# emstoudenmire/TNML

Hardware: AMD Instinct MI355X
Metric: two-site bond updates/sec (higher is better)
Workload: dtype f64; 1 GPU; fixedL N=784, maxm=120, 60000 images (BASELINE config 3: its 60 000 images on 1 GPU instead of 8), Npass=4, lambda=0.001, minm=120, fp64 throughout; random-init W at m=maxm; timed bonds 405..202 (consecutive interior bonds, Label-carrying shiftE on each, m=119); global_images=60000, sites=784, maxm=120, parallelism=dp1 (image sharding + RCCL all-reduce), rccl_ranks=1

## Files before the change

### tnml_amd/csrc/kernels_res.hip

```cpp
#include "tnml_internal.h"

typedef double f64x4r __attribute__((ext_vector_type(4)));

#define FR_TI 32
#define FR_ROWS(NKA) (4 * (NKA) + 4)
#define FR_EIS(NKA) (FR_ROWS(NKA) * FR_TI)
#define FR_LDS_DOUBLES_N(NKA) (2 * FR_EIS(NKA) + 2 * 64 * FR_TI + 2 * 4 * TNML_NL * FR_TI)
#define FR_LDS_DOUBLES FR_LDS_DOUBLES_N(30)

static __device__ __forceinline__ void fr_barrier() {
    asm volatile("s_waitcnt lgkmcnt(0)" ::: "memory");
    __builtin_amdgcn_s_barrier();
    asm volatile("" ::: "memory");
}

template <int PS, int PK, int ABL, int NKA = 30, bool GEN = false, int NST = 8>
__global__ __launch_bounds__(768) void k_fwd_res(FwdResArgs A) {
    static_assert(GEN || NKA == 30, "the constant-extent form is the 120 x 120 bond");
    static_assert(NST == 8 || (NST == 4 && GEN), "four or eight streaming steps per tile");
    constexpr int EIS = FR_EIS(NKA);
    const int mI = GEN ? A.mI : 120, mO = GEN ? A.mO : 120, Kp = GEN ? A.Kp : 240, Np = GEN ? A.Np : 240;
    extern __shared__ __attribute__((aligned(16))) double fr_lds[];
    double* EIs = fr_lds;
    double* Us = EIs + 2 * EIS;
    double* red = Us + 2 * 64 * FR_TI;
    const int tid = threadIdx.x, lane = tid & 63, wid = __builtin_amdgcn_readfirstlane(tid >> 6);
    const int b = blockIdx.x;
    const int half = (b >> 3) & 1, pair = (b & 7) + 8 * (b >> 4), npairs = gridDim.x >> 1;
    const int NTp = A.NTp;
    const int T = Np >> 4, T0 = (T + 1) >> 1;
    const int Th = half ? T - T0 : T0;
    const int qb = half ? 8 * T0 : 0;
    const int niter = (A.ntiles - pair + npairs - 1) / npairs;

    if (wid < 8) {
        const int w = wid;
        const bool act = w < Th;
        const int ct = (half ? T0 : 0) + w;
        double me[NKA], mo[NKA];
        {
            const int g = lane >> 4, i = lane & 15;
            const int col = 2 * (8 * ct + (i & 7)) + (i >> 3);
#pragma unroll
            for (int ks = 0; ks < NKA; ++ks) {
                const bool in = act && 2 * (4 * ks + g) + 1 < Kp;
                me[ks] = in ? A.M[(size_t)(2 * (4 * ks + g)) * Np + col] : 0.;
                mo[ks] = in ? A.M[(size_t)(2 * (4 * ks + g) + 1) * Np + col] : 0.;
            }
        }
        fr_barrier();
        long long t_mma = 0, t_epi = 0, t_bar = 0;
        const long long wc0 = ABL == 5 ? (long long)wall_clock64() : 0;
        for (int it = 0; it < niter + 2; ++it) {
            const long long c0 = ABL == 5 ? clock64() : 0;
            long long c1 = c0, c2 = c0;
            if (it < niter && act) {
                const double* Eb = EIs + (it & 1) * EIS;
                double* Ub = Us + (it & 1) * 64 * FR_TI;
                int ln = lane;
                asm volatile("" : "+v"(ln));
                int g = ln >> 4, i = ln & 15;
                const double* ep0 = Eb + g * FR_TI + 16 * (g & 1) + i;
                const double* ep1 = Eb + g * FR_TI + 16 * ((g & 1) ^ 1) + i;
                f64x4r ce0 = {0., 0., 0., 0.}, co0 = {0., 0., 0., 0.}, ce1 = {0., 0., 0., 0.}, co1 = {0., 0., 0., 0.};
                double a0 = ep0[0], b0 = ep1[0], a1 = ep0[4 * FR_TI], b1 = ep1[4 * FR_TI];
                __builtin_amdgcn_sched_group_barrier(0x100, 4, 0);
#pragma unroll
                for (int ks = 0; ks < (ABL == 2 ? 1 : NKA); ++ks) {
                    const double xa = a0, xb = b0;
                    a0 = a1; b0 = b1;
                    if (ks + 2 < NKA) { a1 = ep0[4 * (ks + 2) * FR_TI]; b1 = ep1[4 * (ks + 2) * FR_TI]; __builtin_amdgcn_sched_group_barrier(0x100, 2, 0); }
                    ce0 = __builtin_amdgcn_mfma_f64_16x16x4f64(me[ks], xa, ce0, 0, 0, 0);
                    co0 = __builtin_amdgcn_mfma_f64_16x16x4f64(mo[ks], xa, co0, 0, 0, 0);
                    ce1 = __builtin_amdgcn_mfma_f64_16x16x4f64(me[ks], xb, ce1, 0, 0, 0);
                    co1 = __builtin_amdgcn_mfma_f64_16x16x4f64(mo[ks], xb, co1, 0, 0, 0);
                    __builtin_amdgcn_sched_group_barrier(0x008, 4, 0);
                    if (PS > 0 && ks % PK == PK - 1) { __builtin_amdgcn_s_sleep(PS); __builtin_amdgcn_sched_barrier(0); }
                }
                if (ABL == 5) c1 = clock64();
                ln = lane;
                asm volatile("" : "+v"(ln));
                g = ln >> 4; i = ln & 15;
#pragma unroll
                for (int grp = 0; grp < 2; ++grp) {
                    const double pI0 = Eb[(4 * NKA) * FR_TI + 16 * grp + i], pI1 = Eb[(4 * NKA + 1) * FR_TI + 16 * (grp ^ 1) + i];
                    const double pO0 = Eb[(4 * NKA + 2) * FR_TI + 16 * grp + i], pO1 = Eb[(4 * NKA + 3) * FR_TI + 16 * (grp ^ 1) + i];
                    const f64x4r ce = grp ? ce1 : ce0, co = grp ? co1 : co0;
#pragma unroll
                    for (int e = 0; e < 2; ++e) {
                        const double t0 = fma(pI1, co[e], pI0 * ce[e]), t1 = fma(pI1, co[e + 2], pI0 * ce[e + 2]);
                        const double v = fma(pO1, t1, pO0 * t0);
                        Ub[(8 * w + g + 4 * e) * FR_TI + 16 * grp + i] = v;
                    }
                }
                if (ABL == 5) c2 = clock64();
            }
            fr_barrier();
            if (ABL == 5) { const long long c3 = clock64(); t_mma += c1 - c0; t_epi += c2 - c1; t_bar += c3 - c2; }
        }
        if (ABL == 5 && A.dbg && blockIdx.x < 16 && lane == 0) { long long* d = A.dbg + (blockIdx.x * 12 + wid) * 4; d[0] = t_mma; d[1] = t_epi; d[2] = t_bar; d[3] = (long long)wall_clock64() - wc0; }
    } else {
        __builtin_amdgcn_s_setprio(3);
        const int sw = wid - 8;
        const int img = lane & 31, qs = lane >> 5;
        const int nk = Th;
        const unsigned lds0 = (unsigned)(size_t)((__attribute__((address_space(3))) char*)fr_lds);
        const int xcol = 2 * ((lane & 15) ^ (((lane >> 4) & 1) << 3));
        const double* const phr = ((lane >> 4) < 2 ? A.phiI : A.phiO) + (size_t)((lane >> 4) & 1) * NTp + xcol;
        const double* const eir = A.EI + (size_t)(lane >> 4) * NTp + xcol;
        const int gb = GEN ? (mI - 1) >> 2 : NKA;
        const int rb = 4 * gb + (lane >> 4) < mI ? 4 * gb + (lane >> 4) : mI - 1;
        const double* const eib = A.EI + (size_t)rb * NTp + xcol;
        auto x_stage = [&](int tile, int buf) {
#pragma unroll
            for (int r = 0; r < 8; ++r) {
                int grp = sw + 4 * r;
                const double* src;
                if constexpr (GEN) {
                    if (grp > NKA) grp -= NKA + 1;
                    if (grp > NKA) grp -= NKA + 1;
                    src = (grp == NKA ? phr : (grp < gb ? eir + (size_t)(4 * grp) * NTp : (grp == gb ? eib : eir))) + (size_t)tile * FR_TI;
                } else {
                    grp = r < 7 ? sw + 4 * r : (sw < 2 ? sw + 28 : (sw == 2 ? 30 : 3));
                    src = (grp == 30 ? phr : eir + (size_t)(4 * grp) * NTp) + (size_t)tile * FR_TI;
                }
                const unsigned dst = lds0 + (unsigned)((buf * EIS + 4 * grp * FR_TI) * sizeof(double));
                unsigned keep;
                asm volatile("s_mov_b32 %0, m0\n\ts_mov_b32 m0, %2\n\ts_nop 0\n\tglobal_load_lds_dwordx4 %1, off\n\ts_mov_b32 m0, %0"
                             : "=&s"(keep) : "v"(src), "s"(dst) : "memory");
            }
        };
        const double* ELw = A.EL + (size_t)(qb + 2 * sw) * NTp;
        const unsigned eoff = (unsigned)(((size_t)qs * NTp + img) * sizeof(double));
        const unsigned uoff = (unsigned)((2 * sw + qs) * FR_TI + img);
        size_t roff[8]; bool same[8];
#pragma unroll
        for (int k = 0; k < 8; ++k) {
            const int q0 = qb + 8 * k + 2 * sw;
            const bool real = k < nk && q0 < mO;
            roff[k] = real ? (size_t)(8 * k) * NTp : (size_t)0 - (size_t)qb * NTp;
            same[k] = GEN && real && q0 + 1 >= mO;
        }
        const unsigned eoff0 = (unsigned)(img * sizeof(double));
        double ea[TNML_NL], eb[TNML_NL], ec[TNML_NL], ed[TNML_NL];
        auto s_load = [&](int tile, int k, double (&e)[TNML_NL]) {
            const unsigned vo = same[k] ? eoff0 : eoff;
#pragma unroll
            for (int l = 0; l < TNML_NL; ++l) {
                const double* bp = ELw + (size_t)tile * FR_TI + (size_t)l * A.EL_lstride + roff[k];
                if (ABL == 1) e[l] = 1.0;
                else asm volatile("global_load_dwordx2 %0, %1, %2 nt" : "=v"(e[l]) : "v"(vo), "s"(bp) : "memory");
            }
        };
#define FR_WAIT(N, e) asm volatile("s_waitcnt vmcnt(" #N ")" : "+v"(e[0]), "+v"(e[1]), "+v"(e[2]), "+v"(e[3]), "+v"(e[4]), "+v"(e[5]), "+v"(e[6]), "+v"(e[7]), "+v"(e[8]), "+v"(e[9]) :: "memory")
        auto label_dot = [&](int tile, int ntile, const double* Ub, double* rb, auto&& mid) {
            double px[TNML_NL];
#pragma unroll
            for (int l = 0; l < TNML_NL; ++l) px[l] = 0.;
            auto s_use = [&](int k, const double (&e)[TNML_NL], bool on) {
                double u = Ub[8 * k * FR_TI + uoff];
                if (!on) u = 0.;
#pragma unroll
                for (int l = 0; l < TNML_NL; ++l) px[l] = fma(e[l], u, px[l]);
            };
#define FR_FENCE() do { asm volatile("" : "+v"(px[0]), "+v"(px[1]), "+v"(px[2]), "+v"(px[3]), "+v"(px[4]), "+v"(px[5]), "+v"(px[6]), "+v"(px[7]), "+v"(px[8]), "+v"(px[9]) :: "memory"); \
                        __builtin_amdgcn_sched_barrier(0); } while (0)
            if constexpr (NST == 8) {
                FR_WAIT(30, ea); s_use(0, ea, nk > 0); FR_FENCE(); s_load(tile, 4, ea);
                FR_WAIT(30, eb); s_use(1, eb, nk > 1); FR_FENCE(); s_load(tile, 5, eb);
                FR_WAIT(30, ec); s_use(2, ec, nk > 2); FR_FENCE(); s_load(tile, 6, ec);
                FR_WAIT(30, ed); s_use(3, ed, nk > 3); FR_FENCE(); s_load(tile, 7, ed);
                mid();
                FR_WAIT(38, ea); s_use(4, ea, nk > 4); FR_FENCE(); s_load(ntile, 0, ea);
                FR_WAIT(38, eb); s_use(5, eb, nk > 5); FR_FENCE(); s_load(ntile, 1, eb);
                FR_WAIT(38, ec); s_use(6, ec, nk > 6); FR_FENCE(); s_load(ntile, 2, ec);
                FR_WAIT(38, ed); s_use(7, ed, nk > 7); FR_FENCE(); s_load(ntile, 3, ed);
            } else {
                FR_WAIT(30, ea); s_use(0, ea, nk > 0); FR_FENCE(); s_load(ntile, 0, ea);
                FR_WAIT(30, eb); s_use(1, eb, nk > 1); FR_FENCE(); s_load(ntile, 1, eb);
                mid();
                FR_WAIT(38, ec); s_use(2, ec, nk > 2); FR_FENCE(); s_load(ntile, 2, ec);
                FR_WAIT(38, ed); s_use(3, ed, nk > 3); FR_FENCE(); s_load(ntile, 3, ed);
            }
#undef FR_FENCE
#pragma unroll
            for (int l = 0; l < TNML_NL; ++l) {
                px[l] += __shfl_xor(px[l], 32);
                if (qs == 0) rb[(sw * TNML_NL + l) * FR_TI + img] = px[l];
            }
        };
        auto finalize = [&](int tile, const double* rb) {
            if (sw == 0) {
#pragma unroll
                for (int l2 = 0; l2 < TNML_NL / 2; ++l2) {
                    const int l = 2 * l2 + qs;
                    const double s = ((rb[(0 * TNML_NL + l) * FR_TI + img] + rb[(1 * TNML_NL + l) * FR_TI + img]) + rb[(2 * TNML_NL + l) * FR_TI + img]) + rb[(3 * TNML_NL + l) * FR_TI + img];
                    A.Ppart[((size_t)half * TNML_NL + l) * NTp + (size_t)tile * FR_TI + img] = s;
                }
            }
        };
        x_stage(pair, 0);
        asm volatile("s_waitcnt vmcnt(0)" ::: "memory");
        fr_barrier();
        x_stage(niter > 1 ? pair + npairs : pair, 1);
        s_load(pair, 0, ea); s_load(pair, 1, eb); s_load(pair, 2, ec); s_load(pair, 3, ed);
        asm volatile("s_waitcnt vmcnt(40)" ::: "memory");
        fr_barrier();
        long long t_dot = 0, t_bar = 0;
        for (int it = 1; it <= niter; ++it) {
            const long long c0 = ABL == 5 ? clock64() : 0;
            const int tile = pair + (it - 1) * npairs;
            label_dot(tile, it < niter ? tile + npairs : tile, Us + ((it - 1) & 1) * 64 * FR_TI, red + (it & 1) * 4 * TNML_NL * FR_TI, [&]() {
                x_stage(it + 1 < niter ? pair + (it + 1) * npairs : tile, (it + 1) & 1);
                if (it >= 2) finalize(pair + (it - 2) * npairs, red + ((it - 1) & 1) * 4 * TNML_NL * FR_TI);
            });
            if constexpr (NST == 8) asm volatile("s_waitcnt vmcnt(40)" ::: "memory");
            else                    asm volatile("s_waitcnt vmcnt(20)" ::: "memory");
            const long long c1 = ABL == 5 ? clock64() : 0;
            fr_barrier();
            if (ABL == 5) { const long long c2 = clock64(); t_dot += c1 - c0; t_bar += c2 - c1; }
        }
        if (ABL == 5 && A.dbg && blockIdx.x < 16 && lane == 0) { long long* d = A.dbg + (blockIdx.x * 12 + wid) * 4; d[0] = t_dot; d[1] = 0; d[2] = t_bar; d[3] = niter; }
        asm volatile("s_waitcnt vmcnt(0)" ::: "memory");
        finalize(pair + (niter - 1) * npairs, red + (niter & 1) * 4 * TNML_NL * FR_TI);
        fr_barrier();
#undef FR_WAIT
    }
}

#define SR_TI 64

template <int NKS, int NG, int NSK>
static __device__ __forceinline__ void sr_groups(const double* Eb, const double (&me)[NKS], const double (&mo)[NKS], int lane, unsigned sl, double (&ob)[16]) {
    int ln = lane;
    asm volatile("" : "+v"(ln));
    int g = ln >> 4;
    const double* ep[NG];
    f64x4r ce[NG], co[NG];
    double x0[NG];
#pragma unroll
    for (int j = 0; j < NG; ++j) {
        ep[j] = Eb + g * SR_TI + ((sl >> (8 * j)) & 63);
        ce[j] = f64x4r{0., 0., 0., 0.}; co[j] = f64x4r{0., 0., 0., 0.};
    }
#pragma unroll
    for (int j = 0; j < NG; ++j) x0[j] = ep[j][0];
    __builtin_amdgcn_sched_group_barrier(0x100, NG, 0);
#pragma unroll
    for (int ks = 0; ks < NKS; ++ks) {
        double xa[NG];
#pragma unroll
        for (int j = 0; j < NG; ++j) xa[j] = x0[j];
        if (ks + 1 < NKS) {
#pragma unroll
            for (int j = 0; j < NG; ++j) x0[j] = ep[j][4 * (ks + 1) * SR_TI];
            __builtin_amdgcn_sched_group_barrier(0x100, NG, 0);
        }
#pragma unroll
        for (int j = 0; j < NG; ++j) {
            ce[j] = __builtin_amdgcn_mfma_f64_16x16x4f64(me[ks], xa[j], ce[j], 0, 0, 0);
            if (j >= NSK) co[j] = __builtin_amdgcn_mfma_f64_16x16x4f64(mo[ks], xa[j], co[j], 0, 0, 0);
        }
        __builtin_amdgcn_sched_group_barrier(0x008, 2 * NG - NSK, 0);
    }
#pragma unroll
    for (int j = 0; j < NG; ++j) {
        const int im = (sl >> (8 * j)) & 63;
        const double pI0 = Eb[(4 * NKS) * SR_TI + im];
        if (j < NSK) {
#pragma unroll
            for (int e = 0; e < 4; ++e) ob[4 * j + e] = pI0 * ce[j][e];
        } else {
            const double pI1 = Eb[(4 * NKS + 1) * SR_TI + im];
#pragma unroll
            for (int e = 0; e < 4; ++e) ob[4 * j + e] = fma(pI1, co[j][e], pI0 * ce[j][e]);
        }
    }
    asm volatile("" ::: "memory");
    __builtin_amdgcn_sched_barrier(0);
}

template <int NKS, bool ZS>
__global__ __launch_bounds__(512) void k_shift_res(ShiftResArgs A) {
    constexpr int ROWS = 4 * NKS + 2;
    constexpr int NP = 2 * NKS + 1;
    extern __shared__ __attribute__((aligned(16))) double sr_lds[];
    const int tid = threadIdx.x, lane = tid & 63, w = __builtin_amdgcn_readfirstlane(tid >> 6);
    const int NTp = A.NTp, tpl = NTp / SR_TI;
    const int G = gridDim.x;
    const int niter = (A.ntiles - (int)blockIdx.x + G - 1) / G;
    const unsigned lds0 = __builtin_amdgcn_readfirstlane((unsigned)(size_t)((__attribute__((address_space(3))) char*)sr_lds));
    const unsigned doff = (unsigned)(((size_t)(lane >> 5) * NTp + 2 * (lane & 31)) * sizeof(double));
    auto dma16 = [&](const double* base, unsigned voff, unsigned dst) {
        unsigned keep;
        asm volatile("s_mov_b32 %0, m0\n\ts_mov_b32 m0, %2\n\ts_nop 0\n\tglobal_load_lds_dwordx4 %1, %3\n\ts_mov_b32 m0, %0" : "=&s"(keep) : "v"(voff), "s"(dst), "s"(base) : "memory");
    };
    const unsigned doff0 = (unsigned)((2 * (lane & 31)) * sizeof(double));
    auto stage = [&](int t, int buf) {
        const int l = t / tpl, n0 = (t - l * tpl) * SR_TI;
        const double* eb = A.EI + (size_t)l * A.EI_lstride + n0;
#pragma unroll
        for (int r = 0; r < 8; ++r) {
            int p = w + 8 * r;
            if (p >= NP) p -= NP;
            if (p >= NP) p -= NP;
            const int r0 = 2 * p < A.mI ? 2 * p : 0;
            dma16(p == NP - 1 ? A.phiI + n0 : eb + (size_t)r0 * NTp, (p != NP - 1 && 2 * p == A.mI - 1) ? doff0 : doff, lds0 + (unsigned)((buf * ROWS * SR_TI + 2 * p * SR_TI) * sizeof(double)));
        }
    };
    const int CT = A.Np >> 4;
    const bool split = CT <= 4;
    const int ct = split ? (w & 3) : w;
    const bool act = ct < CT;
    const bool do0 = !split || w < 4, do1 = !split || w >= 4;
    double me[NKS], mo[NKS];
    {
        const int g = lane >> 4, i = lane & 15;
#pragma unroll
        for (int ks = 0; ks < NKS; ++ks) {
            const bool in = act && 2 * (4 * ks + g) + 1 < A.Kp;
            me[ks] = in ? A.M[(size_t)(2 * (4 * ks + g)) * A.Np + 16 * ct + i] : 0.;
            mo[ks] = in ? A.M[(size_t)(2 * (4 * ks + g) + 1) * A.Np + 16 * ct + i] : 0.;
        }
    }
    if (niter > 0) stage(blockIdx.x, 0);
    asm volatile("s_waitcnt vmcnt(0)" ::: "memory");
    fr_barrier();
    if constexpr (ZS) {
        auto slots = [&](int t, int ln) {
            const uint8_t* o = A.ord + (size_t)(t % tpl) * SR_TI + (ln & 15);
            return (unsigned)o[0] | (unsigned)o[16] << 8 | (unsigned)o[32] << 16 | (unsigned)o[48] << 24;
        };
        auto put = [&](int t, int ln, unsigned psl, const double (&ob)[16]) {
            const int l = t / tpl, n0 = (t - l * tpl) * SR_TI, g = ln >> 4;
            double* op = A.out + (size_t)l * A.out_lstride + (size_t)(16 * ct + g) * NTp + n0;
#pragma unroll
            for (int q = 0; q < 16; ++q) {
                const int y = 16 * ct + g + 4 * (q & 3);
                if (y < A.mO && (q < 8 || !split)) op[(size_t)(4 * (q & 3)) * NTp + ((psl >> (8 * (q >> 2))) & 63)] = ob[q];
            }
        };
        unsigned sl = 0, sln = 0, psl = 0;
        if (niter > 0) sl = slots(blockIdx.x, lane);
        double ob[16];
        for (int it = 0; it < niter; ++it) {
            const int t = blockIdx.x + it * G;
            int ln = lane;
            asm volatile("" : "+v"(ln));
            if (act && it > 0) put(t - G, ln, psl, ob);
            if (it + 1 < niter) { stage(t + G, (it + 1) & 1); sln = slots(t + G, ln); }
            const double* Eb = sr_lds + (it & 1) * ROWS * SR_TI;
            if (act) {
                const int s = __builtin_amdgcn_readfirstlane((int)(((sl >> 6) & 3) | ((sl >> 12) & 4)));
                if (!split) {
                    switch (s) {
                        case 0:  sr_groups<NKS, 4, 0>(Eb, me, mo, lane, sl, ob); break;
                        case 1:  sr_groups<NKS, 4, 1>(Eb, me, mo, lane, sl, ob); break;
                        case 2:  sr_groups<NKS, 4, 2>(Eb, me, mo, lane, sl, ob); break;
                        case 3:  sr_groups<NKS, 4, 3>(Eb, me, mo, lane, sl, ob); break;
                        default: sr_groups<NKS, 4, 4>(Eb, me, mo, lane, sl, ob); break;
                    }
                    psl = sl;
                } else {
                    const int s2 = w < 4 ? (s < 2 ? s : 2) : (s > 2 ? s - 2 : 0);
                    psl = w < 4 ? sl : sl >> 16;
                    switch (s2) {
                        case 0:  sr_groups<NKS, 2, 0>(Eb, me, mo, lane, psl, ob); break;
                        case 1:  sr_groups<NKS, 2, 1>(Eb, me, mo, lane, psl, ob); break;
                        default: sr_groups<NKS, 2, 2>(Eb, me, mo, lane, psl, ob); break;
                    }
                }
            }
            asm volatile("s_waitcnt vmcnt(0)" : "+v"(sln) :: "memory");
            sl = sln;
            fr_barrier();
        }
        if (act && niter > 0) put(blockIdx.x + (niter - 1) * G, lane, psl, ob);
        return;
    }
    double ob[8];
    double* obp = nullptr;
    for (int it = 0; it < niter; ++it) {
        const int t = blockIdx.x + it * G;
        const int l = t / tpl, n0 = (t - l * tpl) * SR_TI;
        int ln = lane;
        asm volatile("" : "+v"(ln));
        int g = ln >> 4, i = ln & 15;
        if (obp) {
#pragma unroll
            for (int q = 0; q < 8; ++q) { const int y = 16 * ct + g + 4 * (q & 3); if (y < A.mO) obp[(size_t)(4 * (q & 3)) * NTp + 16 * (q >> 2)] = ob[q]; }
        }
        if (it + 1 < niter) stage(t + G, (it + 1) & 1);
        const double* Eb = sr_lds + (it & 1) * ROWS * SR_TI;
        double* op = A.out + (size_t)l * A.out_lstride + (size_t)(16 * ct + g) * NTp + n0 + i;
        if (act) {
#pragma unroll
            for (int pass = 0; pass < 2; ++pass) {
                if (pass == 0 ? !do0 : !do1) continue;
                const double* ep0 = Eb + g * SR_TI + 32 * pass + i;
                const double* ep1 = ep0 + 16;
                f64x4r ce0 = {0., 0., 0., 0.}, co0 = {0., 0., 0., 0.}, ce1 = {0., 0., 0., 0.}, co1 = {0., 0., 0., 0.};
                double a0 = ep0[0], b0 = ep1[0], a1 = ep0[4 * SR_TI], b1 = ep1[4 * SR_TI];
                __builtin_amdgcn_sched_group_barrier(0x100, 4, 0);
#pragma unroll
                for (int ks = 0; ks < NKS; ++ks) {
                    const double xa = a0, xb = b0;
                    a0 = a1; b0 = b1;
                    if (ks + 2 < NKS) { a1 = ep0[4 * (ks + 2) * SR_TI]; b1 = ep1[4 * (ks + 2) * SR_TI]; __builtin_amdgcn_sched_group_barrier(0x100, 2, 0); }
                    ce0 = __builtin_amdgcn_mfma_f64_16x16x4f64(me[ks], xa, ce0, 0, 0, 0);
                    co0 = __builtin_amdgcn_mfma_f64_16x16x4f64(mo[ks], xa, co0, 0, 0, 0);
                    ce1 = __builtin_amdgcn_mfma_f64_16x16x4f64(me[ks], xb, ce1, 0, 0, 0);
                    co1 = __builtin_amdgcn_mfma_f64_16x16x4f64(mo[ks], xb, co1, 0, 0, 0);
                    __builtin_amdgcn_sched_group_barrier(0x008, 4, 0);
                }
                ln = lane;
                asm volatile("" : "+v"(ln));
                g = ln >> 4; i = ln & 15;
#pragma unroll
                for (int grp = 0; grp < 2; ++grp) {
                    const double pI0 = Eb[(4 * NKS) * SR_TI + 32 * pass + 16 * grp + i], pI1 = Eb[(4 * NKS + 1) * SR_TI + 32 * pass + 16 * grp + i];
#pragma unroll
                    for (int e = 0; e < 4; ++e) {
                        const double v = fma(pI1, grp ? co1[e] : co0[e], pI0 * (grp ? ce1[e] : ce0[e]));
                        if (pass == 0) { if (16 * ct + g + 4 * e < A.mO) op[(size_t)(4 * e) * NTp + 16 * grp] = v; }
                        else ob[4 * grp + e] = v;
                    }
                }
                asm volatile("" ::: "memory");
                __builtin_amdgcn_sched_barrier(0);
            }
            if (do1) obp = op + 32;
        }
        asm volatile("s_waitcnt vmcnt(0)" ::: "memory");
        fr_barrier();
    }
    if (obp) {
        const int g = lane >> 4;
#pragma unroll
        for (int q = 0; q < 8; ++q) { const int y = 16 * ct + g + 4 * (q & 3); if (y < A.mO) obp[(size_t)(4 * (q & 3)) * NTp + 16 * (q >> 2)] = ob[q]; }
    }
}

static const int sr_nks_list[] = {12, 16, 18, 20, 22, 24, 26, 28, 30};
static int sr_nks_for(int mI) {
    for (int v : sr_nks_list) if (4 * v >= mI) return v;
    return 0;
}
bool shift_res_applies(int mI, int mO) { return mI >= 33 && sr_nks_for(mI) != 0 && mO >= 1 && mO <= 128; }

template <int NKS>
static int shift_res_go(tnml_ctx* c, const ShiftResArgs& a, int grid) {
    const size_t lds = sizeof(double) * 2 * (4 * NKS + 2) * SR_TI;
    if (!c->attr_sr[NKS]) {
        if (hipFuncSetAttribute(reinterpret_cast<const void*>(k_shift_res<NKS, false>), hipFuncAttributeMaxDynamicSharedMemorySize, (int)lds) != hipSuccess ||
            hipFuncSetAttribute(reinterpret_cast<const void*>(k_shift_res<NKS, true>), hipFuncAttributeMaxDynamicSharedMemorySize, (int)lds) != hipSuccess)
            return tnml_fail(c, "shift_res: cannot reserve %zu bytes of LDS", lds);
        c->attr_sr[NKS] = true;
    }
    ProfScope ps(c, KC_FGEMM_SHIFT);
    if (a.ord && a.nz) hipLaunchKernelGGL((k_shift_res<NKS, true>), dim3(grid), dim3(512), lds, c->stream, a);
    else               hipLaunchKernelGGL((k_shift_res<NKS, false>), dim3(grid), dim3(512), lds, c->stream, a);
    return 0;
}
int launch_shift_res(tnml_ctx* c, const ShiftResArgs& a_in) {
    ShiftResArgs a = a_in;
    if (a.NTp % SR_TI) return tnml_fail(c, "shift_res: image count not a multiple of %d", SR_TI);
    if (((size_t)a.L * a.EI_lstride) * sizeof(double) >= ((size_t)1 << 32)) return tnml_fail(c, "shift_res: environment larger than 4 GB (32-bit lane offsets)");
    if (!shift_res_applies(a.mI, a.mO) || a.Np % 16 || a.Np < a.mO || a.Np > 128) return tnml_fail(c, "shift_res: bond dimensions %d x %d (packed %d) not served", a.mI, a.mO, a.Np);
    if (!c->cu_count) { hipDeviceProp_t pr; c->cu_count = hipGetDeviceProperties(&pr, c->cfg.device) == hipSuccess ? pr.multiProcessorCount : 256; }
    a.ntiles = a.L * (a.NTp / SR_TI);
    int grid = c->cu_count;
    if (c->res_grid > 0 && c->res_grid < grid) grid = c->res_grid;
    if (grid > a.ntiles) grid = a.ntiles;
    switch (sr_nks_for(a.mI)) {
        case 12: TCK((shift_res_go<12>(c, a, grid))); break;
        case 16: TCK((shift_res_go<16>(c, a, grid))); break;
        case 18: TCK((shift_res_go<18>(c, a, grid))); break;
        case 20: TCK((shift_res_go<20>(c, a, grid))); break;
        case 22: TCK((shift_res_go<22>(c, a, grid))); break;
        case 24: TCK((shift_res_go<24>(c, a, grid))); break;
        case 26: TCK((shift_res_go<26>(c, a, grid))); break;
        case 28: TCK((shift_res_go<28>(c, a, grid))); break;
        default: TCK((shift_res_go<30>(c, a, grid))); break;
    }
    HIPCK(c, hipGetLastError());
    return 0;
}

__global__ __launch_bounds__(256) void k_shift_order(const double* __restrict__ phi, int N, int NTp, uint8_t* __restrict__ ord, uint8_t* __restrict__ nz, int* __restrict__ cnt) {
    const int lane = threadIdx.x & 63, tpl = NTp / SR_TI;
    const size_t wave = (size_t)blockIdx.x * 4 + (threadIdx.x >> 6);
    if (wave >= (size_t)N * tpl) return;
    const int j = (int)(wave / tpl), ti = (int)(wave - (size_t)j * tpl);
    const bool z = phi[((size_t)j * 2 + 1) * NTp + (size_t)ti * SR_TI + lane] == 0.0;
    const unsigned long long mz = __ballot(z), below = ((unsigned long long)1 << lane) - 1;
    const int nzc = __popcll(mz);
    const int slot = z ? __popcll(mz & below) : nzc + __popcll(~mz & below);
    const int sk = nzc >> 4, code = slot < 16 ? (sk & 3) : (slot < 32 ? sk >> 2 : 0);
    ord[((size_t)j * tpl + ti) * SR_TI + slot] = (uint8_t)(lane | code << 6);
    if (lane == 0) { nz[(size_t)j * tpl + ti] = (uint8_t)nzc; if (nzc >= 16) atomicAdd(cnt + j, nzc >> 4); }
}
int launch_shift_order(tnml_ctx* c, const double* phi, int N, int NTp, uint8_t* ord, uint8_t* nz, int* cnt) {
    if (NTp % SR_TI) return tnml_fail(c, "shift_order: image count not a multiple of %d", SR_TI);
    ProfScope ps(c, KC_PACK);
    HIPCK(c, hipMemsetAsync(cnt, 0, sizeof(int) * N, c->stream));
    const size_t waves = (size_t)N * (NTp / SR_TI);
    hipLaunchKernelGGL(k_shift_order, dim3((unsigned)((waves + 3) / 4)), dim3(256), 0, c->stream, phi, N, NTp, ord, nz, cnt);
    HIPCK(c, hipGetLastError());
    return 0;
}

static __device__ __forceinline__ void res_wave_partials(double val, int lab, int cor, bool pap, double* out, int lane) {
    if (pap) {
        const double s = wave_sum(val);
        if (lane < 12) out[lane] = lane == 11 ? s : 0.;
        return;
    }
    double mine = 0.;
#pragma unroll
    for (int t = 0; t < TNML_NL; ++t) {
        const double s = wave_sum(lab == t ? val : 0.);
        if (lane == t) mine = s;
    }
    const double sc = wave_sum((double)cor);
    if (lane == 10) mine = sc;
    if (lane < 12) out[lane] = mine;
}

__global__ __launch_bounds__(256) void k_pfinish(PfinishArgs A) {
    const int tid = threadIdx.x, lane = tid & 63;
    const int NTp = A.NTp;
    const int ni = blockIdx.x * 256 + tid;
    if (A.conv && A.conv[0] != 0.) return;
    const int lab = A.label[ni];
    double P[TNML_NL];
    if (A.npart == 2) {
#pragma unroll
        for (int l = 0; l < TNML_NL; ++l) P[l] = A.Ppart[(size_t)l * NTp + ni] + A.Ppart[((size_t)TNML_NL + l) * NTp + ni];
    } else {
        const double a = A.alpha[0];
#pragma unroll
        for (int l = 0; l < TNML_NL; ++l) P[l] = fma(a, A.Pp[(size_t)l * NTp + ni], A.P[(size_t)l * NTp + ni]);
    }
    double val = 0.; int cor = 0;
    if (A.mode == LD_MODE_PAP) {
#pragma unroll
        for (int l = 0; l < TNML_NL; ++l) {
            val = fma(P[l], P[l], val);
            if (A.Pout) A.Pout[(size_t)l * NTp + ni] = P[l];
        }
        if (lab < 0) val = 0.;
    } else {
        double best = fabs(P[0]); int arg = 0;
#pragma unroll
        for (int l = 0; l < TNML_NL; ++l) {
            const double tgt = l == lab ? 1. : 0.;
            const double d = lab >= 0 ? tgt - P[l] : 0.;
            val = fma(d, d, val);
            if (A.dP) A.dP[(size_t)l * NTp + ni] = d;
            if (A.Pout) A.Pout[(size_t)l * NTp + ni] = P[l];
            const double wgt = fabs(P[l]);
            if (wgt > best) { best = wgt; arg = l; }
        }
        cor = (lab >= 0 && arg == lab) ? 1 : 0;
    }
    res_wave_partials(val, lab, cor, A.mode == LD_MODE_PAP, A.partials + ((size_t)blockIdx.x * 4 + (tid >> 6)) * 12, lane);
}

template <int PS, int PK, int NKA, bool GEN, int NST = 8>
static int fwd_res_go(tnml_ctx* c, const FwdResArgs& a, int grid) {
    const size_t lds = sizeof(double) * FR_LDS_DOUBLES_N(NKA);
    bool& done = c->attr_fr[2 * (GEN ? 1 : 0) + (NST == 4 ? 1 : 0)][NKA];
    if (!done || !GEN) {
        if (hipFuncSetAttribute(reinterpret_cast<const void*>(k_fwd_res<PS, PK, 0, NKA, GEN, NST>), hipFuncAttributeMaxDynamicSharedMemorySize, (int)lds) != hipSuccess)
            return tnml_fail(c, "fwd_res: cannot reserve %zu bytes of LDS", lds);
        done = true;
    }
    ProfScope ps(c, KC_FWD_RES);
    hipLaunchKernelGGL((k_fwd_res<PS, PK, 0, NKA, GEN, NST>), dim3(grid), dim3(768), lds, c->stream, a);
    return 0;
}
static const int fr_nka_list[] = {12, 16, 18, 20, 22, 24, 26, 28, 30};
static int fr_nka_for(int mI) {
    for (int v : fr_nka_list) if (4 * v >= mI) return v;
    return 0;
}
bool fwd_res_applies(int mI, int mO) { return mI >= 33 && fr_nka_for(mI) != 0 && mO >= 16 && mO <= 120; }
int launch_fwd_res(tnml_ctx* c, const FwdResArgs& a) {
    if (a.NTp % 256) return tnml_fail(c, "fwd_res: image count not a multiple of 256");
    if ((size_t)TNML_NL * a.EL_lstride * sizeof(double) >= ((size_t)1 << 32)) return tnml_fail(c, "fwd_res: environment larger than 4 GB (32-bit lane offsets)");
    if (!fwd_res_applies(a.mI, a.mO) || a.Np % 16 || a.Np < 2 * a.mO || a.Np > 240 || a.Kp < 2 * a.mI) return tnml_fail(c, "fwd_res: bond %d x %d (packed %d x %d) not served", a.mI, a.mO, a.Kp, a.Np);
    if (!c->cu_count) { hipDeviceProp_t pr; c->cu_count = hipGetDeviceProperties(&pr, c->cfg.device) == hipSuccess ? pr.multiProcessorCount : 256; }
    int grid = c->cu_count / 16 * 16;
    if (c->res_grid > 0 && c->res_grid < grid) grid = c->res_grid / 16 * 16;
    if (grid < 16) grid = 16;
    while (grid > 16 && (grid / 2) > a.ntiles) grid -= 16;
    if (a.mI == 120 && a.mO == 120 && a.Kp == 240 && a.Np == 240 && c->fwd_res != 3) {
        switch (c->res_pace) {
            case 1:  TCK((fwd_res_go<0, 1, 30, false>(c, a, grid))); break;
            case 2:  TCK((fwd_res_go<4, 2, 30, false>(c, a, grid))); break;
            case 3:  TCK((fwd_res_go<6, 3, 30, false>(c, a, grid))); break;
            case 4:  TCK((fwd_res_go<4, 1, 30, false>(c, a, grid))); break;
            default: TCK((fwd_res_go<6, 2, 30, false>(c, a, grid))); break;
        }
    } else if (a.Np <= 128) {
        switch (fr_nka_for(a.mI)) {
            case 12: TCK((fwd_res_go<6, 2, 12, true, 4>(c, a, grid))); break;
            case 16: TCK((fwd_res_go<6, 2, 16, true, 4>(c, a, grid))); break;
            case 18: TCK((fwd_res_go<6, 2, 18, true, 4>(c, a, grid))); break;
            case 20: TCK((fwd_res_go<6, 2, 20, true, 4>(c, a, grid))); break;
            case 22: TCK((fwd_res_go<6, 2, 22, true, 4>(c, a, grid))); break;
            case 24: TCK((fwd_res_go<6, 2, 24, true, 4>(c, a, grid))); break;
            case 26: TCK((fwd_res_go<6, 2, 26, true, 4>(c, a, grid))); break;
            case 28: TCK((fwd_res_go<6, 2, 28, true, 4>(c, a, grid))); break;
            default: TCK((fwd_res_go<6, 2, 30, true, 4>(c, a, grid))); break;
        }
    } else {
        switch (fr_nka_for(a.mI)) {
            case 12: TCK((fwd_res_go<6, 2, 12, true>(c, a, grid))); break;
            case 16: TCK((fwd_res_go<6, 2, 16, true>(c, a, grid))); break;
            case 18: TCK((fwd_res_go<6, 2, 18, true>(c, a, grid))); break;
            case 20: TCK((fwd_res_go<6, 2, 20, true>(c, a, grid))); break;
            case 22: TCK((fwd_res_go<6, 2, 22, true>(c, a, grid))); break;
            case 24: TCK((fwd_res_go<6, 2, 24, true>(c, a, grid))); break;
            case 26: TCK((fwd_res_go<6, 2, 26, true>(c, a, grid))); break;
            case 28: TCK((fwd_res_go<6, 2, 28, true>(c, a, grid))); break;
            default: TCK((fwd_res_go<6, 2, 30, true>(c, a, grid))); break;
        }
    }
    HIPCK(c, hipGetLastError());
    return 0;
}
int launch_pfinish(tnml_ctx* c, const PfinishArgs& a) {
    if (a.NTp % 256) return tnml_fail(c, "pfinish: image count not a multiple of 256");
    ProfScope ps(c, KC_PUPDATE);
    hipLaunchKernelGGL(k_pfinish, dim3(a.NTp / 256), dim3(256), 0, c->stream, a);
    HIPCK(c, hipGetLastError());
    return 0;
}
```

Baseline: 407.0 bond updates/s.

## Restructure shift kernel: runtime skip count, deeper LDS prefetch, mid-loop staging

The templated sr_groups switch over skip counts becomes one sr_round that takes the skip count s at runtime. Under the default macros, the next tile's DMA staging and slot loads are issued halfway through the MFMA loop through a callback, the pI scale factors are read early, and the M fragments are pinned in registers. The aim is to overlap global-to-LDS traffic with compute and to cut code-size and branch overhead. Several probe macros, including an include file under tools/probe, are added but are off by default, and the runtime s check adds a branch inside the MFMA loop.

Measured after the change: 403.1 bond updates/s. No clear change (-1.0%).

```diff
diff --git a/tnml_amd/csrc/kernels_res.hip b/tnml_amd/csrc/kernels_res.hip
--- a/tnml_amd/csrc/kernels_res.hip
+++ b/tnml_amd/csrc/kernels_res.hip
@@ -230,50 +230,120 @@
 
 #define SR_TI 64
 
-template <int NKS, int NG, int NSK>
-static __device__ __forceinline__ void sr_groups(const double* Eb, const double (&me)[NKS], const double (&mo)[NKS], int lane, unsigned sl, double (&ob)[16]) {
+#ifndef SR_BODY_SWITCH
+#define SR_BODY_SWITCH 0
+#endif
+#ifndef SR_PIN_M
+#define SR_PIN_M 1
+#endif
+#ifndef SR_SLOTS_JOIN
+#define SR_SLOTS_JOIN 0
+#endif
+#ifndef SR_STAGE_MID
+#define SR_STAGE_MID 1
+#endif
+#ifndef SR_PI_EARLY
+#define SR_PI_EARLY 1
+#endif
+#ifndef SR_PF
+#define SR_PF 1
+#endif
+#ifndef SR_ORDER_IL
+#define SR_ORDER_IL 0
+#endif
+#ifndef SR_STORE_SPLIT
+#define SR_STORE_SPLIT 0
+#endif
+#ifndef SR_ORD_PAIRS
+#define SR_ORD_PAIRS 0
+#endif
+#ifndef SR_NOSKIP
+#define SR_NOSKIP 0
+#endif
+#ifndef SR_NAT_READS
+#define SR_NAT_READS 0
+#endif
+#ifndef SR_NAT_STORES
+#define SR_NAT_STORES 0
+#endif
+#ifndef SR_ABL
+#define SR_ABL 0
+#endif
+#if SR_BODY_SWITCH
+#include "../../tools/probe/sr_groups_switch.inc"
+#endif
+
+template <int NKS, int NG, class MID>
+static __device__ __forceinline__ void sr_round(const double* Eb, const double (&me)[NKS], const double (&mo)[NKS], int lane, unsigned sl, int s, double (&ob)[16], MID&& mid) {
+    constexpr int PF = SR_PF;
     int ln = lane;
     asm volatile("" : "+v"(ln));
     int g = ln >> 4;
     const double* ep[NG];
     f64x4r ce[NG], co[NG];
-    double x0[NG];
+    double x[PF][NG], pI0[NG], pI1[NG];
 #pragma unroll
     for (int j = 0; j < NG; ++j) {
-        ep[j] = Eb + g * SR_TI + ((sl >> (8 * j)) & 63);
+        ep[j] = Eb + g * SR_TI + (SR_NAT_READS ? 16 * j + (ln & 15) : (int)((sl >> (8 * j)) & 63));
         ce[j] = f64x4r{0., 0., 0., 0.}; co[j] = f64x4r{0., 0., 0., 0.};
     }
 #pragma unroll
-    for (int j = 0; j < NG; ++j) x0[j] = ep[j][0];
-    __builtin_amdgcn_sched_group_barrier(0x100, NG, 0);
+    for (int d = 0; d < PF; ++d)
+#pragma unroll
+        for (int j = 0; j < NG; ++j) x[d][j] = ep[j][4 * d * SR_TI];
+    __builtin_amdgcn_sched_group_barrier(0x100, PF * NG, 0);
 #pragma unroll
     for (int ks = 0; ks < NKS; ++ks) {
         double xa[NG];
 #pragma unroll
-        for (int j = 0; j < NG; ++j) xa[j] = x0[j];
-        if (ks + 1 < NKS) {
-#pragma unroll
-            for (int j = 0; j < NG; ++j) x0[j] = ep[j][4 * (ks + 1) * SR_TI];
+        for (int j = 0; j < NG; ++j) {
+            xa[j] = x[0][j];
+#pragma unroll
+            for (int d = 0; d + 1 < PF; ++d) x[d][j] = x[d + 1][j];
+        }
+        if (ks + PF < NKS) {
+#pragma unroll
+            for (int j = 0; j < NG; ++j) x[PF - 1][j] = ep[j][4 * (ks + PF) * SR_TI];
             __builtin_amdgcn_sched_group_barrier(0x100, NG, 0);
         }
+#if SR_ORDER_IL
 #pragma unroll
         for (int j = 0; j < NG; ++j) {
             ce[j] = __builtin_amdgcn_mfma_f64_16x16x4f64(me[ks], xa[j], ce[j], 0, 0, 0);
-            if (j >= NSK) co[j] = __builtin_amdgcn_mfma_f64_16x16x4f64(mo[ks], xa[j], co[j], 0, 0, 0);
-        }
-        __builtin_amdgcn_sched_group_barrier(0x008, 2 * NG - NSK, 0);
+            if (j >= s) co[j] = __builtin_amdgcn_mfma_f64_16x16x4f64(mo[ks], xa[j], co[j], 0, 0, 0);
+        }
+#else
+#pragma unroll
+        for (int j = 0; j < NG; ++j) ce[j] = __builtin_amdgcn_mfma_f64_16x16x4f64(me[ks], xa[j], ce[j], 0, 0, 0);
+        __builtin_amdgcn_sched_group_barrier(0x008, NG, 0);
+#pragma unroll
+        for (int j = NG - 1; j >= 0; --j) {
+            if (j < s) break;
+            co[j] = __builtin_amdgcn_mfma_f64_16x16x4f64(mo[ks], xa[j], co[j], 0, 0, 0);
+        }
+#endif
+        if (ks == NKS / 2 - 1) mid();
+        if (SR_PI_EARLY && ks == NKS - PF) {
+#pragma unroll
+            for (int j = 0; j < NG; ++j) pI0[j] = Eb[(4 * NKS) * SR_TI + ((sl >> (8 * j)) & 63)];
+        }
+        if (SR_PI_EARLY && ks == NKS - 1) {
+#pragma unroll
+            for (int j = 0; j < NG; ++j) pI1[j] = Eb[(4 * NKS + 1) * SR_TI + ((sl >> (8 * j)) & 63)];
+        }
     }
 #pragma unroll
     for (int j = 0; j < NG; ++j) {
-        const int im = (sl >> (8 * j)) & 63;
-        const double pI0 = Eb[(4 * NKS) * SR_TI + im];
-        if (j < NSK) {
-#pragma unroll
-            for (int e = 0; e < 4; ++e) ob[4 * j + e] = pI0 * ce[j][e];
+        if (!SR_PI_EARLY) {
+            pI0[j] = Eb[(4 * NKS) * SR_TI + ((sl >> (8 * j)) & 63)];
+            pI1[j] = Eb[(4 * NKS + 1) * SR_TI + ((sl >> (8 * j)) & 63)];
+        }
+        if (j < s) {
+#pragma unroll
+            for (int e = 0; e < 4; ++e) ob[4 * j + e] = pI0[j] * ce[j][e];
         } else {
-            const double pI1 = Eb[(4 * NKS + 1) * SR_TI + im];
-#pragma unroll
-            for (int e = 0; e < 4; ++e) ob[4 * j + e] = fma(pI1, co[j][e], pI0 * ce[j][e]);
+#pragma unroll
+            for (int e = 0; e < 4; ++e) ob[4 * j + e] = fma(pI1[j], co[j][e], pI0[j] * ce[j][e]);
         }
     }
     asm volatile("" ::: "memory");
@@ -331,51 +401,73 @@
             const uint8_t* o = A.ord + (size_t)(t % tpl) * SR_TI + (ln & 15);
             return (unsigned)o[0] | (unsigned)o[16] << 8 | (unsigned)o[32] << 16 | (unsigned)o[48] << 24;
         };
-        auto put = [&](int t, int ln, unsigned psl, const double (&ob)[16]) {
+        auto put = [&](int t, int ln, unsigned psl, const double (&ob)[16], int q0, int q1) {
             const int l = t / tpl, n0 = (t - l * tpl) * SR_TI, g = ln >> 4;
             double* op = A.out + (size_t)l * A.out_lstride + (size_t)(16 * ct + g) * NTp + n0;
 #pragma unroll
             for (int q = 0; q < 16; ++q) {
                 const int y = 16 * ct + g + 4 * (q & 3);
-                if (y < A.mO && (q < 8 || !split)) op[(size_t)(4 * (q & 3)) * NTp + ((psl >> (8 * (q >> 2))) & 63)] = ob[q];
+                const int im = SR_NAT_STORES ? 16 * (q >> 2) + (ln & 15) + (split && w >= 4 ? 32 : 0) : (int)((psl >> (8 * (q >> 2))) & 63);
+                if (q >= q0 && q < q1 && y < A.mO && (q < 8 || !split)) op[(size_t)(4 * (q & 3)) * NTp + im] = ob[q];
             }
         };
-        unsigned sl = 0, sln = 0, psl = 0;
+        constexpr int QTOP = SR_STORE_SPLIT && !SR_BODY_SWITCH ? 8 : 16;
+        unsigned sl = 0, psl = 0, sb0 = 0, sb1 = 0, sb2 = 0, sb3 = 0;
         if (niter > 0) sl = slots(blockIdx.x, lane);
+#if SR_PIN_M
+#pragma unroll
+        for (int ks = 0; ks < NKS; ++ks) asm volatile("" : "+v"(me[ks]), "+v"(mo[ks]));
+        asm volatile("" : "+v"(sl));
+#endif
         double ob[16];
         for (int it = 0; it < niter; ++it) {
             const int t = blockIdx.x + it * G;
             int ln = lane;
             asm volatile("" : "+v"(ln));
-            if (act && it > 0) put(t - G, ln, psl, ob);
-            if (it + 1 < niter) { stage(t + G, (it + 1) & 1); sln = slots(t + G, ln); }
+            if (act && it > 0) put(t - G, ln, psl, ob, 0, QTOP);
+            auto next = [&](int l2) {
+                if (it + 1 < niter) {
+                    if (SR_ABL != 2) stage(t + G, (it + 1) & 1);
+                    const uint8_t* o = A.ord + (size_t)((t + G) % tpl) * SR_TI + (l2 & 15);
+                    sb0 = o[0]; sb1 = o[16]; sb2 = o[32]; sb3 = o[48];
+#if SR_SLOTS_JOIN
+                    sb0 = sb0 | sb1 << 8 | sb2 << 16 | sb3 << 24; sb1 = sb2 = sb3 = 0;
+#endif
+                }
+            };
+            constexpr bool NEXT_MID = SR_STAGE_MID && !SR_BODY_SWITCH;
+            if (!NEXT_MID || !act) next(ln);
             const double* Eb = sr_lds + (it & 1) * ROWS * SR_TI;
             if (act) {
-                const int s = __builtin_amdgcn_readfirstlane((int)(((sl >> 6) & 3) | ((sl >> 12) & 4)));
+                const int s = SR_NOSKIP && NTp > 0 ? 0 : __builtin_amdgcn_readfirstlane((int)(((sl >> 6) & 3) | ((sl >> 12) & 4)));
+#if SR_BODY_SWITCH
+                psl = sr_round_switch<NKS>(Eb, me, mo, lane, sl, s, split, w, ob);
+#else
                 if (!split) {
-                    switch (s) {
-                        case 0:  sr_groups<NKS, 4, 0>(Eb, me, mo, lane, sl, ob); break;
-                        case 1:  sr_groups<NKS, 4, 1>(Eb, me, mo, lane, sl, ob); break;
-                        case 2:  sr_groups<NKS, 4, 2>(Eb, me, mo, lane, sl, ob); break;
-                        case 3:  sr_groups<NKS, 4, 3>(Eb, me, mo, lane, sl, ob); break;
-                        default: sr_groups<NKS, 4, 4>(Eb, me, mo, lane, sl, ob); break;
-                    }
+                    const unsigned osl = psl;
+                    sr_round<NKS, 4>(Eb, me, mo, lane, sl, s, ob, [&]() {
+                        int l2 = lane;
+                        asm volatile("" : "+v"(l2));
+                        if (QTOP < 16 && it > 0) put(t - G, l2, osl, ob, QTOP, 16);
+                        if (NEXT_MID) next(l2);
+                    });
                     psl = sl;
                 } else {
                     const int s2 = w < 4 ? (s < 2 ? s : 2) : (s > 2 ? s - 2 : 0);
                     psl = w < 4 ? sl : sl >> 16;
-                    switch (s2) {
-                        case 0:  sr_groups<NKS, 2, 0>(Eb, me, mo, lane, psl, ob); break;
-                        case 1:  sr_groups<NKS, 2, 1>(Eb, me, mo, lane, psl, ob); break;
-                        default: sr_groups<NKS, 2, 2>(Eb, me, mo, lane, psl, ob); break;
-                    }
+                    sr_round<NKS, 2>(Eb, me, mo, lane, psl, s2, ob, [&]() {
+                        int l2 = lane;
+                        asm volatile("" : "+v"(l2));
+                        if (NEXT_MID) next(l2);
+                    });
                 }
-            }
-            asm volatile("s_waitcnt vmcnt(0)" : "+v"(sln) :: "memory");
-            sl = sln;
+#endif
+            }
+            asm volatile("s_waitcnt vmcnt(0)" : "+v"(sb0), "+v"(sb1), "+v"(sb2), "+v"(sb3) :: "memory");
+            sl = sb0 | sb1 << 8 | sb2 << 16 | sb3 << 24;
             fr_barrier();
         }
-        if (act && niter > 0) put(blockIdx.x + (niter - 1) * G, lane, psl, ob);
+        if (act && niter > 0) put(blockIdx.x + (niter - 1) * G, lane, psl, ob, 0, 16);
         return;
     }
     double ob[8];
@@ -495,7 +587,16 @@
     const bool z = phi[((size_t)j * 2 + 1) * NTp + (size_t)ti * SR_TI + lane] == 0.0;
     const unsigned long long mz = __ballot(z), below = ((unsigned long long)1 << lane) - 1;
     const int nzc = __popcll(mz);
-    const int slot = z ? __popcll(mz & below) : nzc + __popcll(~mz & below);
+    int slot;
+    if (!SR_ORD_PAIRS) slot = z ? __popcll(mz & below) : nzc + __popcll(~mz & below);
+    else {
+        const unsigned long long mc = z ? mz : ~mz;
+        const unsigned long long lo = mc & (mc >> 32) & 0xffffffffull, up = lo << 32;
+        const unsigned long long single = mc & ~(lo | up);
+        const int np = __popcll(lo), ns = __popcll(single);
+        const int idx = (lo >> lane) & 1 ? __popcll(lo & below) : ((single >> lane) & 1 ? np + __popcll(single & below) : np + ns + __popcll(up & below));
+        slot = z ? idx : 63 - idx;
+    }
     const int sk = nzc >> 4, code = slot < 16 ? (sk & 3) : (slot < 32 ? sk >> 2 : 0);
     ord[((size_t)j * tpl + ti) * SR_TI + slot] = (uint8_t)(lane | code << 6);
     if (lane == 0) { nz[(size_t)j * tpl + ti] = (uint8_t)nzc; if (nzc >= 16) atomicAdd(cnt + j, nzc >> 4); }
```
